# nygenome/Lancet2

Hardware: AMD Instinct MI355X
Metric: microassembly windows/sec (whole node) (higher is better)
Workload: dtype u8/i32 (f64 statistics)

## Files before the change

### lancet2_amd/csrc/build.hip

```cpp
#include "graph_ws.h"

namespace ma {

constexpr int kBT = 256;
__constant__ u64 c_phred_bits[256] = {
#include "../../include/ma_phred_lut.inc"
};

struct SeqInfo {
  u64 off;
  u32 len;
  u32 nk;
};

__device__ __forceinline__ u32 seq_count(const DBatch& b, int w) {
  return 1u + (b.read_win_off[w + 1] - b.read_win_off[w]);
}

__device__ __forceinline__ SeqInfo seq_info(const DBatch& b, int w, u32 s, int k) {
  SeqInfo si;
  if (s == 0) {
    si.off = b.ref_off[w];
    si.len = b.ref_off[w + 1] - b.ref_off[w];
  } else {
// ... 689 lines not shown
      u32 const x = x0 + u * kInsT;
      live[u] = x < nq;
      item[u] = live[u] ? slowq[x] : 0u;
    }
#pragma unroll
    for (int u = 0; u < kIU; ++u) {
      u32 const s_idx = (item[u] >> 12) & kQSeqMask, o = item[u] & 0xFFFu;
      if (staged) {
        off[u] = live[u] ? l_rpos[s_idx] + o : 0u;
        inst[u] = live[u] ? l_ibase[s_idx] + o : 0u;
      } else {
        SeqInfo const si = seq_info(b, w, live[u] ? s_idx : 0u, k);
        off[u] = si.off + o;
        inst[u] = live[u] ? ws.seq_inst_base[base_idx + s_idx] + o : 0u;
      }
    }
#pragma unroll
    for (int u = 0; u < kIU; ++u) {
      id[u] = 1;
      plus[u] = true;
      if (live[u])
        id[u] = staged ? kmer_id_lds(l_seq, static_cast<u32>(off[u]), k, &plus[u]) : kmer_id(b.read_bases + off[u], k, &plus[u]);
    }
#pragma unroll
    for (int u = 0; u < kIU; ++u) {
      if (!live[u]) continue;
      recs[rsi.nk + x0 + u * kInsT] = make_uint4(static_cast<u32>(id[u]), static_cast<u32>(id[u] >> 32),
                                                 inst[u] | (item[u] & (kQErrFree | kQLast)) | (plus[u] ? kQPlus : 0u),
                                                 (item[u] >> 12) & kQSeqMask);
    }
  }
  __threadfence_block();
  __syncthreads();
  IPROF(1);
  auto map_entry = [&](u64 id) -> u32 {
    u32 e = static_cast<u32>(id >> 32) % kInsMap;
    u32 const lim = *reinterpret_cast<volatile u32*>(&l_nmap) + 64u >= kInsMap ? 64u : kInsProbe;
    for (u32 probe = 0; probe < lim; ++probe) {
      u64 cur = l_key[e];
      if (cur == 0) {
        unsigned long long const old = atomicCAS(reinterpret_cast<unsigned long long*>(&l_key[e]), 0ull,
                                                 static_cast<unsigned long long>(id));
        if (old == 0ull) atomicAdd(&l_nmap, 1u);
        cur = old == 0ull ? id : old;
      }
      if (cur == id) return e;
      e = e + 1 == kInsMap ? 0u : e + 1;
    }
    return kNoNode;
  };
  auto map_find = [&](u64 id) -> u32 {
    u32 e = static_cast<u32>(id >> 32) % kInsMap;
    for (u32 probe = 0; probe < kInsProbe; ++probe) {
      u64 const cur = l_key[e];
      if (cur == id) return e;
      if (cur == 0) return kNoNode;
      e = e + 1 == kInsMap ? 0u : e + 1;
    }
    return kNoNode;
  };
  auto const word_flags = [](u32 z) -> u32 {
    return ((z & kQPlus) ? kInstPlus : 0u) | ((z & kQErrFree) ? kInstErrFree : 0u) | ((z & kQLast) ? kInstLast : 0u);
  };
  auto const rec_id = [](uint4 const& r) -> u64 { return static_cast<u64>(r.x) | (static_cast<u64>(r.y) << 32); };
  int const CW = ws.num_samples + 2;
  u32* cnt = ws.tbl_cnt + (static_cast<size_t>(a) << tcl) * CW;
  auto map_pass = [&](u32 ncls, u32 cls) {
    __syncthreads();
    for (u32 i = threadIdx.x; i < kInsMap; i += kInsT) {
      l_key[i] = 0;
      l_min[i] = 0xFFFFFFFFu;
    }
    if (threadIdx.x == 0) l_nmap = 0;
    __syncthreads();
    u32 const sbase = cls * kInsMap;
    for (u32 p = threadIdx.x; p < rsi.nk; p += kInsT) {
      uint4 const rc = recs[p];
      if (ncls > 1 && (rc.x & 0xFFFFu) % ncls != cls) continue;
      u32 const e = map_entry(rec_id(rc));
      if (e != kNoNode) {
        atomicMin(&l_min[e], p);
        inst_slot[p] = (sbase + e) | word_flags(rc.z);
        ref_slot_g[p] = sbase + e;
      } else {
        atomicAdd(&l_ndef, 1u);
      }
    }
    __syncthreads();
    for (u32 x0 = threadIdx.x; x0 < nq; x0 += kInsT * kIU) {
      uint4 rc[kIU];
      bool live[kIU];
#pragma unroll
      for (int u = 0; u < kIU; ++u) {
        u32 const x = x0 + u * kInsT;
        live[u] = x < nq;
        rc[u] = recs[rsi.nk + (live[u] ? x : 0u)];
      }
#pragma unroll
      for (int u = 0; u < kIU; ++u) {
        if (!live[u] || (ncls > 1 && (rc[u].x & 0xFFFFu) % ncls != cls)) continue;
        u32 const e = map_entry(rec_id(rc[u]));
        if (e != kNoNode) {
          u32 const inst = rc[u].z & kInstIdx;
          u32 const before = atomicMin(&l_min[e], inst);
          inst_slot[inst] = (sbase + e) | word_flags(rc[u].z);
          if ((rc[u].z & kQErrFree) && before < rsi.nk) ws.rd_flag[r_first + rc[u].w - 1] = 1;
        } else {
          atomicAdd(&l_ndef, 1u);
        }
      }
    }
    __syncthreads();
  };
  auto copy_out = [&](u32 cls) {
    for (u32 i = threadIdx.x; i < kInsMap; i += kInsT) {
      u64 const id = l_key[i];
      keys[cls * kInsMap + i] = id;
      first[cls * kInsMap + i] = id ? l_min[i] : 0x7F7F7F7Fu;
    }
  };
  map_pass(1, 0);
  IPROF(3);
  if (l_ndef == 0 && (1u << tcl) >= kInsMap) {
    copy_out(0);
    for (u32 i = threadIdx.x; i < kInsMap * CW; i += kInsT) cnt[i] = 0;
    if (threadIdx.x == 0) ws.win_nslots[a] = kInsMap;
    IPROF(4);
    return;
  }
  {
    u32 const ndef0 = l_ndef;
    u32 ncls = 2;
    while (ncls < 16u && (kInsMap + ndef0 / 4u) > ncls * (kInsMap * 6u / 10u)) ncls *= 2u;
    bool tried = false;
    while (ndef0 && ncls <= 16u && (1u << tcl) >= ncls * kInsMap) {
      tried = true;
      __syncthreads();
      if (threadIdx.x == 0) l_ndef = 0;
      for (u32 cls = 0; cls < ncls; ++cls) {
        map_pass(ncls, cls);
        if (l_ndef != 0) break;
        copy_out(cls);
      }
      if (l_ndef == 0) {
        for (u32 i = threadIdx.x; i < ncls * kInsMap * CW; i += kInsT) cnt[i] = 0;
        if (threadIdx.x == 0) ws.win_nslots[a] = ncls * kInsMap;
        return;
      }
      ncls *= 2u;
    }
    if (tried) {
      __syncthreads();
      if (threadIdx.x == 0) l_ndef = 0;
      map_pass(1, 0);
    }
  }
  u32 nslots;
  {
    u32 tcw = 10;
    while (tcw < static_cast<u32>(tcl) && (1u << tcw) < (l_nmap + l_ndef) * 4u / 3u + 16u) ++tcw;
    nslots = 1u << tcw;
  }
  u32 const mask = nslots - 1;
  for (u32 i = threadIdx.x; i < nslots; i += kInsT) {
    keys[i] = 0ull;
    first[i] = 0x7F7F7F7Fu;
  }
  for (u32 i = threadIdx.x; i < nslots * CW; i += kInsT) cnt[i] = 0;
  if (threadIdx.x == 0) ws.win_nslots[a] = nslots;
  __syncthreads();
  for (u32 e = threadIdx.x; e < kInsMap; e += kInsT) {
    u64 const id = l_key[e];
    if (id == 0) continue;
    u32 const slot = table_insert(keys, mask, id, &ws.win_flags[w]);
    u32 const fi = l_min[e];
    if (slot == kNoNode) atomicOr(&ws.win_flags[w], 4u);
    else first[slot] = fi;
    l_min[e] = (slot == kNoNode ? 0x7FFFFFFFu : (slot & kInstSlotMask)) | (fi < rsi.nk ? 0x80000000u : 0u);
  }
  __syncthreads();
  auto direct_insert = [&](u64 id, u32 inst, u32* old_first) -> u32 {
    u32 const slot = table_insert(keys, mask, id, &ws.win_flags[w]);
    *old_first = 0xFFFFFFFFu;
    if (slot == kNoNode) {
      atomicOr(&ws.win_flags[w], 4u);
      return 0u;
    }
    *old_first = atomicMin(&first[slot], inst);
    return slot & kInstSlotMask;
  };
  for (u32 p = threadIdx.x; p < rsi.nk; p += kInsT) {
    uint4 const rc = recs[p];
    u32 const e = map_find(rec_id(rc));
    u32 slot, of;
    if (e != kNoNode) {
      slot = l_min[e] & 0x7FFFFFFFu;
      if (slot == 0x7FFFFFFFu) slot = 0u; else atomicMin(&first[slot], p);
    } else {
      slot = direct_insert(rec_id(rc), p, &of);
    }
    inst_slot[p] = word_flags(rc.z) | slot;
    ref_slot_g[p] = slot;
  }
  __syncthreads();
  for (u32 x = threadIdx.x; x < nq; x += kInsT) {
    uint4 const rc = recs[rsi.nk + x];
    u32 const inst = rc.z & kInstIdx;
    u32 const e = map_find(rec_id(rc));
    u32 slot;
    bool isref;
    if (e != kNoNode) {
      u32 const sv = l_min[e];
      slot = sv & 0x7FFFFFFFu;
      if (slot == 0x7FFFFFFFu) slot = 0u; else atomicMin(&first[slot], inst);
      isref = (sv >> 31) != 0;
    } else {
      u32 of;
      slot = direct_insert(rec_id(rc), inst, &of);
      isref = of < rsi.nk;
    }
    inst_slot[inst] = slot | word_flags(rc.z);
    if ((rc.z & kQErrFree) && isref) ws.rd_flag[r_first + rc.w - 1] = 1;
  }
  IPROF(5);
}
__global__ __launch_bounds__(kInsT) __attribute__((amdgpu_waves_per_eu(8, 8))) void k_insert(DBatch b, GraphWs ws) {
  __shared__ __align__(16) unsigned char l_area[12u * kInsMapA];
  insert_window<kInsMapA, kInsStageA>(b, ws, static_cast<int>(blockIdx.x), l_area);
}
#ifdef MA_PROFILE
extern "C" void ma_debug_iprof(unsigned long long* out) { (void)hipMemcpyFromSymbol(out, HIP_SYMBOL(g_iprof), sizeof(unsigned long long) * 32); }
#endif

constexpr u32 kGrSlots = 6144;
__device__ __forceinline__ u32 edge_word(u32 word) { return ((word & kInstFast) ? (1u << 20) : 0u) | (word & 0xFFFFFu); }
__device__ __forceinline__ uint2 edge_pack(u32 ii, u32 wa, u32 wb) {
  u32 const ca = edge_word(wa), cb = edge_word(wb);
  return make_uint2((ii & 0x3FFFFFu) | (ca << 22), (ca >> 10) | (cb << 11));
}
constexpr u32 kSupCache = 2048;
constexpr int kSupT = 512;
__global__ __launch_bounds__(kSupT) void k_support(DBatch b, GraphWs ws, u32* max_gen, u32 cache_cap, u32 xs_log2) {
  extern __shared__ unsigned char lds_build[];
  __shared__ u32 xs_flag;
  __shared__ u32 any_big;
  __shared__ u32 gen_count;
  __shared__ u32 genq_n;
  __shared__ u32 edgeq_n;
  __shared__ u32 n_leaders;
  int const a = blockIdx.x;
  int const w = static_cast<int>(ws.active[a]);
  int const k = win_kmer(ws, w);
  int const S = ws.num_samples, CW = S + 2;
  u32* gcnt = ws.tbl_cnt + (static_cast<size_t>(a) << tbl_log2(ws)) * CW;
  u32* inst_slot = ws.inst_slot + static_cast<size_t>(a) * ws.inst_stride;
  const u32* ref_slot_g = ws.ref_slot + static_cast<size_t>(a) * ws.ref_stride;
  u32 const ns = seq_count(b, w);
  u32 const base_idx = b.read_win_off[w] + w;
  u32 off = 0;
  u32* l_cnt = reinterpret_cast<u32*>(lds_build + off);
  u32 const cnt_words = (ws.ref_stride * CW + 1u) / 2u;
  off += 4u * cnt_words;
  u32* l_dd = reinterpret_cast<u32*>(lds_build + off);
  off += 4u * (kSupT / 64u) << ws.dd_log2;
  u32* l_mask = reinterpret_cast<u32*>(lds_build + off);
  off += 4u * (ws.max_reads + 2u);
  u32 const xs_cap = 1u << xs_log2, xs_shift = 32u - xs_log2;
  u32* l_xkey = reinterpret_cast<u32*>(lds_build + off);
  off += 4u * xs_cap;
  u32* l_xgrp = reinterpret_cast<u32*>(lds_build + off);
  off += 4u * xs_cap;
  u8* l_xsmp = lds_build + off;
  off = (off + xs_cap + 15u) & ~15u;
  u32* c_meta = reinterpret_cast<u32*>(lds_build + off);
  u32* c_qn = c_meta + cache_cap;
  u32* c_ib = c_qn + cache_cap;
  i32* c_hint = reinterpret_cast<i32*>(c_ib + cache_cap);
  bool const cached = cache_cap != 0 && ns <= cache_cap;
  SeqInfo const rsi = seq_info(b, w, 0, k);
  for (u32 i = threadIdx.x; i < cnt_words; i += kSupT) l_cnt[i] = 0;
  for (u32 i = threadIdx.x; i < (kSupT / 64u) << ws.dd_log2; i += kSupT) l_dd[i] = 0;
  for (u32 i = threadIdx.x; i < xs_cap; i += kSupT) {
    l_xkey[i] = 0;
    l_xgrp[i] = 0;
  }
  if (threadIdx.x == 0) {
    xs_flag = ns > 65535u ? 1u : 0u;
    any_big = 0;
    gen_count = 0;
    genq_n = 0;
    edgeq_n = 0;
  }
  if (cached) {
    for (u32 sx = 1 + threadIdx.x; sx < ns; sx += kSupT) {
      u32 const r = b.read_win_off[w] + sx - 1;
      SeqInfo const si = seq_info(b, w, sx, k);
      c_meta[sx] = (b.read_flags[r] & 7u) | (ws.rd_flag[r] ? 8u : 0u) | (static_cast<u32>(b.read_sample[r]) << 8) | (min(si.nk, 0xFFFFu) << 16);
      c_qn[sx] = b.read_qname_id[r];
      c_ib[sx] = ws.seq_inst_base[base_idx + sx];
      c_hint[sx] = b.read_hint ? b.read_hint[r] : 0;
    }
  }
  __syncthreads();
  bool const hints = b.read_hint != nullptr && rsi.len <= ws.max_ref_len + 8;
  if (hints) {
    for (u32 s_idx = 1 + threadIdx.x; s_idx < ns; s_idx += kSupT) {
      u32 const r = b.read_win_off[w] + s_idx - 1;
      if (!(b.read_flags[r] & MA_RF_PASS)) continue;
      u32 const key = ((b.read_qname_id[r] << 1) | ((b.read_flags[r] & MA_RF_CASE) ? 1u : 0u)) + 1u;
      u32 h = (key * 2654435761u) >> xs_shift;
      bool done = false;
      for (u32 probe = 0; probe < xs_cap && !done; ++probe) {
        u32 cur = l_xkey[h];
        if (cur == 0) {
          u32 const old = atomicCAS(&l_xkey[h], 0u, key);
          if (old == 0) {
            l_xsmp[h] = b.read_sample[r];
            done = true;
            break;
          }
          cur = old;
        }
        if (cur == key) done = true; else h = (h + 1) & (xs_cap - 1);
      }
      if (!done) xs_flag = 1;
    }
  }
  __syncthreads();
  if (hints) {
    for (u32 s_idx = 1 + threadIdx.x; s_idx < ns; s_idx += kSupT) {
      u32 const r = b.read_win_off[w] + s_idx - 1;
      if (!(b.read_flags[r] & MA_RF_PASS)) continue;
      bool const leader = !(s_idx > 1 && same_group(b, r, r - 1));
      u32 const key = ((b.read_qname_id[r] << 1) | ((b.read_flags[r] & MA_RF_CASE) ? 1u : 0u)) + 1u;
      u32 h = (key * 2654435761u) >> xs_shift;
      for (u32 probe = 0; probe < xs_cap; ++probe) {
        u32 const cur = l_xkey[h];
        if (cur == key) {
          if (l_xsmp[h] != b.read_sample[r]) xs_flag = 1;
          if (leader && atomicAdd(&l_xgrp[h], 1u) != 0) xs_flag = 1;
          break;
        }
        if (cur == 0) break;
        h = (h + 1) & (xs_cap - 1);
      }
    }
  }
  if (hints && ns > kSeqCap) {
    for (u32 s_idx = 1 + kMmRunMax + threadIdx.x; s_idx < ns; s_idx += kSupT) {
      u32 const r = b.read_win_off[w] + s_idx - 1;
      u32 j = 0;
      while (j < kMmRunMax && same_group(b, r - j, r - j - 1)) ++j;
      if (j == kMmRunMax) xs_flag = 1;
    }
  }
  __syncthreads();
  bool const all_generic = !hints || xs_flag != 0;
  bool const qmode = !all_generic && !ws.mm_force_hbm && ns <= kSeqCap && tbl_log2(ws) <= 20;
  u32* const genq = ws.slowq + static_cast<size_t>(a) * ws.inst_stride;
  u32 const dd_cap = 1u << ws.dd_log2;
  uint2* const edgeq = reinterpret_cast<uint2*>(ws.slow_rec + static_cast<size_t>(a) * ws.inst_stride);

  u32* const l_leaders = l_mask;
  if (threadIdx.x == 0) n_leaders = 0;
  __syncthreads();
  for (u32 s_idx = 1 + threadIdx.x; s_idx < ns; s_idx += kSupT) {
    u32 const r0 = b.read_win_off[w] + s_idx - 1;
    if (!(b.read_flags[r0] & MA_RF_PASS)) continue;
    if (s_idx > 1 && same_group(b, r0, r0 - 1)) continue;
    l_leaders[atomicAdd(&n_leaders, 1u)] = s_idx;
    if (qmode) {
      u32 tot = 0;
      for (u32 j = 0; s_idx + j < ns && (j == 0 || same_group(b, r0, r0 + j)); ++j) tot += seq_info(b, w, s_idx + j, k).nk;
      if (tot > dd_cap / 4u * 3u) any_big = 1;
    }
  }
  __syncthreads();
  bool const qdedup = qmode && ws.graph_fused && !any_big && ws.win_nslots[a] <= kGrSlots;
  IPROF_T0();
  u32 const wave = threadIdx.x >> 6, lane = threadIdx.x & 63u;
  u32* const dd = l_dd + (wave << ws.dd_log2);
  u32 wave_gen = 0;
  auto same_group_c = [&](u32 sa, u32 sb) {
    u32 const ma_ = c_meta[sa], mb = c_meta[sb];
    return (mb & MA_RF_PASS) && c_qn[sa] == c_qn[sb] && ((ma_ ^ mb) & MA_RF_CASE) == 0 && ((ma_ ^ mb) & 0xFF00u) == 0;
  };
  for (u32 gi = wave; gi < n_leaders; gi += kSupT / 64) {
    u32 const s_idx = l_leaders[gi];
    u32 const r0 = b.read_win_off[w] + s_idx - 1;
    u32 gsize = 1;
    if (cached) {
      while (s_idx + gsize < ns && same_group_c(s_idx, s_idx + gsize)) gsize++;
    } else {
      while (s_idx + gsize < ns && same_group(b, r0, r0 + gsize)) gsize++;
    }
    bool generic = all_generic || gsize > 2;
    for (u32 gm = 0; gm < gsize && !generic; ++gm) {
      if (cached) {
        u32 const mt = c_meta[s_idx + gm];
        if ((mt & 8u) || (mt >> 16) > 32u * kMaskWords) generic = true;
      } else {
        SeqInfo const si = seq_info(b, w, s_idx + gm, k);
        if (ws.rd_flag[r0 + gm] || si.nk > 32u * kMaskWords) generic = true;
      }
    }
    u32 pre00 = 0, pre01 = 0, pre10 = 0, pre11 = 0;
    bool have_pre = cached && gsize <= 2;
    for (u32 gm = 0; gm < gsize && have_pre; ++gm) {
      u32 const nkc = c_meta[s_idx + gm] >> 16;
      if (nkc == 0xFFFFu || nkc > 128u) have_pre = false;
    }
    if (have_pre) {
      u32 const nka = c_meta[s_idx] >> 16, iba = c_ib[s_idx];
      pre00 = lane < nka ? inst_slot[iba + lane] : 0u;
      pre01 = 64u + lane < nka ? inst_slot[iba + 64u + lane] : 0u;
      if (gsize == 2) {
        u32 const nkb = c_meta[s_idx + 1] >> 16, ibb = c_ib[s_idx + 1];
        pre10 = lane < nkb ? inst_slot[ibb + lane] : 0u;
        pre11 = 64u + lane < nkb ? inst_slot[ibb + 64u + lane] : 0u;
      }
    }
    i32 hint0 = 0;
    u32 nk0 = 0;
    unsigned long long m0[kMaskWords / 2];
#pragma unroll
    for (int x = 0; x < kMaskWords / 2; ++x) m0[x] = 0;
    for (u32 gm = 0; gm < gsize; ++gm) {
      u32 const sx = s_idx + gm;
      u32 const r = r0 + gm;
      SeqInfo si;
      u32 ibase, smp, role;
      i32 hint_r;
      if (cached && (c_meta[sx] >> 16) != 0xFFFFu) {
        u32 const mt = c_meta[sx];
        si.nk = mt >> 16;
        ibase = c_ib[sx];
        smp = (mt >> 8) & 0xFFu;
        role = (mt & MA_RF_CASE) ? 1u : 0u;
        hint_r = c_hint[sx];
      } else {
        si = seq_info(b, w, sx, k);
        ibase = ws.seq_inst_base[base_idx + sx];
        smp = b.read_sample[r];
        role = (b.read_flags[r] & MA_RF_CASE) ? 1u : 0u;
        hint_r = hints ? b.read_hint[r] : 0;
      }
      if (si.nk == 0) continue;
      if (smp >= static_cast<u32>(S)) smp = S - 1;
      if (gm == 0) {
        hint0 = hints ? hint_r : 0;
        nk0 = si.nk;
      }
      for (u32 ob = 0; ob < si.nk; ob += 64) {
        u32 const o = ob + lane;
        u32 const word = have_pre ? (gm == 0 ? (ob == 0 ? pre00 : pre01) : (ob == 0 ? pre10 : pre11))
                                  : (o < si.nk ? inst_slot[ibase + o] : 0u);
        {
          u32 const dn = __shfl_down(word, 1, 64);
          u32 first_next;
          if (have_pre) first_next = ob == 0 ? __shfl(gm == 0 ? pre01 : pre11, 0, 64) : 0u;
          else first_next = ob + 64 < si.nk ? inst_slot[ibase + ob + 64] : 0u;
          u32 const nextw = lane == 63 ? first_next : dn;
          bool const pair = o + 1 < si.nk && !((word & kInstFast) && (nextw & kInstFast) &&
                                               (nextw & kInstSlotMask) == (word & kInstSlotMask) + 1u);
          unsigned long long const em = __ballot(pair);
          if (em) {
            u32 eb = 0;
            if (lane == 0) eb = atomicAdd(&edgeq_n, static_cast<u32>(__popcll(em)));
            eb = __shfl(eb, 0, 64);
            if (pair) edgeq[eb + static_cast<u32>(__popcll(em & ((1ull << lane) - 1ull)))] = edge_pack(ibase + o, word, nextw);
          }
        }
        bool const ef = (word & kInstErrFree) != 0;
        bool const to_gen = ef && (generic || !(word & kInstFast));
        u32 const p = word & kInstSlotMask;
        unsigned long long const gmask = __ballot(to_gen);
        if (qdedup) {
          if (gmask) {
            u32 const nslot = to_gen ? ((word & kInstFast) ? ref_slot_g[p] : p) : 0u;
            bool won = false;
            if (to_gen) {
              u32 const tag = gi + 1u, mine = (nslot << 11) | tag;
              u32 h = (nslot * 2654435761u) >> (32u - ws.dd_log2);
              for (;;) {
                u32 cur = dd[h];
                if ((cur & 0x7FFu) != tag) {
                  u32 const old = atomicCAS(&dd[h], cur, mine);
                  if (old == cur) {
                    won = true;
                    break;
                  }
                  cur = old;
                  if ((cur & 0x7FFu) != tag) continue;
                }
                if (cur == mine) break;
                h = (h + 1u) & (dd_cap - 1u);
              }
            }
            unsigned long long const wm = __ballot(won);
            if (wm) {
              u32 qb = 0;
              if (lane == 0) qb = atomicAdd(&genq_n, static_cast<u32>(__popcll(wm)));
              qb = __shfl(qb, 0, 64);
              if (won) genq[qb + static_cast<u32>(__popcll(wm & ((1ull << lane) - 1ull)))] = (nslot << 4) | (smp << 1) | role;
            }
          }
        } else if (qmode) {
          if (gmask) {
            u32 qb = 0;
            if (lane == 0) qb = atomicAdd(&genq_n, static_cast<u32>(__popcll(gmask)));
            qb = __shfl(qb, 0, 64);
            if (to_gen) {
              u32 const nslot = (word & kInstFast) ? ref_slot_g[p] : p;
              genq[qb + static_cast<u32>(__popcll(gmask & ((1ull << lane) - 1ull)))] = ((nslot << 11) | (s_idx - 1u)) + 1u;
            }
          }
        } else if (to_gen) {
          inst_slot[ibase + o] = word | kInstGen;
        }
        wave_gen += static_cast<u32>(__popcll(gmask));
        bool const fast = ef && !to_gen;
        bool dup = false;
        if (gm == 1 && nk0 > 0 && fast) {
          i64 const o0 = static_cast<i64>(p) - hint0;
          if (o0 >= 0 && o0 < static_cast<i64>(nk0)) {
            unsigned long long wd = 0;
#pragma unroll
            for (int x = 0; x < kMaskWords / 2; ++x) wd = (o0 >> 6) == x ? m0[x] : wd;
            dup = (wd >> (o0 & 63)) & 1ull;
          }
        }
        if (gm == 0 && !generic) {
          unsigned long long const cm = __ballot(fast);
#pragma unroll
          for (int x = 0; x < kMaskWords / 2; ++x)
            if (static_cast<int>(ob >> 6) == x) m0[x] = cm;
        }
        if (fast && !dup) {
          u32 const i1 = p * CW + smp, i2 = p * CW + S + role;
          atomicAdd(&l_cnt[i1 >> 1], 1u << ((i1 & 1u) * 16u));
          atomicAdd(&l_cnt[i2 >> 1], 1u << ((i2 & 1u) * 16u));
        }
      }
    }
  }
  if (lane == 0 && wave_gen) atomicAdd(&gen_count, wave_gen);
  IPROF_SYNC(27);
  if (threadIdx.x == 0) {
    bool const lds_ok = !all_generic && !ws.mm_force_hbm && (ns > kSeqCap || gen_count <= 4u * kMmLdsMax) && tbl_log2(ws) <= 20;
    ws.n_edgeq[a] = edgeq_n;
    ws.n_genq[a] = (qmode || qdedup) ? genq_n : 0u;
    ws.mm_mode[a] = qdedup ? (gen_count | 0x20000000u) : qmode ? (gen_count | 0x40000000u) : (gen_count | (lds_ok ? 0u : 0x80000000u));
    atomic_max_lazy(max_gen, gen_count);
    ws.mm_log2[a] = 0;
    if (!qmode && !lds_ok && gen_count) {
      atomic_max_lazy(max_gen + 1, gen_count);
      u32 lg = 10;
      while (lg < 31u && (1ull << lg) < static_cast<u64>(gen_count) * 4u / 3u + 16u) ++lg;
      unsigned long long const bytes = ((12ull << lg) + 255ull) & ~255ull;
      unsigned long long const at = atomicAdd(ws.mm_pool_used, bytes);
      if (at + bytes <= ws.mm_pool_bytes) {
        ws.mm_off[a] = at;
        ws.mm_log2[a] = lg;
      } else {
        atomicOr(&ws.win_flags[w], 4u);
      }
    }
  }
  for (u32 i = threadIdx.x; i < rsi.nk * CW; i += kSupT) {
    u32 const v = (l_cnt[i >> 1] >> ((i & 1u) * 16u)) & 0xFFFFu;
    if (v == 0) continue;
    u32 const p = i / CW, x = i % CW;
    atomicAdd(&gcnt[static_cast<size_t>(ref_slot_g[p]) * CW + x], v);
  }
  IPROF(28);
}

__device__ __forceinline__ u64 mm_key_of(u32 slot, u32 qname, u32 role) {
  return ((static_cast<u64>(slot) << 33) | (static_cast<u64>(qname) << 1) | role) + 1ull;
}
__device__ __forceinline__ u32 inst_table_slot(u32 word, const u32* ref_slot_g) {
  return (word & kInstFast) ? ref_slot_g[word & kInstSlotMask] : (word & kInstSlotMask);
}

__device__ __forceinline__ void mm_hbm_insert(DBatch const& b, GraphWs const& ws, int a, u32* l_base) {
  if (!(ws.mm_mode[a] & 0x80000000u) || ws.mm_log2[a] == 0) return;
  int const w = static_cast<int>(ws.active[a]);
  u32 const mlg = ws.mm_log2[a];
  u32 const mask = (1u << mlg) - 1;
  u64* keys = reinterpret_cast<u64*>(ws.mm_pool + ws.mm_off[a]);
  u32* mins = reinterpret_cast<u32*>(keys + (size_t(1) << mlg));
  const u32* inst_slot = ws.inst_slot + static_cast<size_t>(a) * ws.inst_stride;
  const u32* ref_slot_g = ws.ref_slot + static_cast<size_t>(a) * ws.ref_stride;
  u32 const ns = seq_count(b, w);
  u32 const base_idx = b.read_win_off[w] + w;
  const u32* sbase = stage_seq_bases(ws.seq_inst_base + base_idx, ns, l_base);
  for (u32 i = threadIdx.x; i < (1u << mlg) / 2u; i += kBT) reinterpret_cast<uint4*>(keys)[i] = make_uint4(0, 0, 0, 0);
  for (u32 i = threadIdx.x; i < (1u << mlg) / 4u; i += kBT)
    reinterpret_cast<uint4*>(mins)[i] = make_uint4(0xFFFFFFFFu, 0xFFFFFFFFu, 0xFFFFFFFFu, 0xFFFFFFFFu);
  __threadfence_block();
  __syncthreads();
  u32 const ninst = ws.win_ninst[w], nref = ninst - ws.win_nread_inst[w];
  for (u32 ii = nref + threadIdx.x; ii < ninst; ii += kBT) {
    u32 const v = inst_slot[ii];
    if ((v & (kInstErrFree | kInstGen)) != (kInstErrFree | kInstGen)) continue;
    u32 const s_idx = seq_of(sbase, ns, ii);
    u32 const r = b.read_win_off[w] + s_idx - 1;
    u32 const qn = b.read_qname_id[r];
    u32 const role = (b.read_flags[r] & MA_RF_CASE) ? 1u : 0u;
    u64 const key = mm_key_of(inst_table_slot(v, ref_slot_g), qn, role);
    u32 slot = static_cast<u32>(dev_fmix64(key)) & mask;
    for (u32 probe = 0; probe <= mask; ++probe) {
      u64 cur = keys[slot];
      if (cur != key && cur == 0) {
        unsigned long long old = atomicCAS(reinterpret_cast<unsigned long long*>(&keys[slot]), 0ull,
                                           static_cast<unsigned long long>(key));
        cur = (old == 0ull) ? key : old;
      }
      if (cur == key) {
        atomicMin(&mins[slot], ii);
        break;
      }
      slot = (slot + 1) & mask;
    }
  }
}

__device__ __forceinline__ void mm_hbm_count(DBatch const& b, GraphWs const& ws, int a, u32* l_base) {
  if (!(ws.mm_mode[a] & 0x80000000u) || ws.mm_log2[a] == 0) return;
  int const w = static_cast<int>(ws.active[a]);
  int const S = ws.num_samples, CW = S + 2;
  u32 const mlg = ws.mm_log2[a];
  u32 const mask = (1u << mlg) - 1;
  const u64* keys = reinterpret_cast<const u64*>(ws.mm_pool + ws.mm_off[a]);
  const u32* mins = reinterpret_cast<const u32*>(keys + (size_t(1) << mlg));
  u32* cnt = ws.tbl_cnt + (static_cast<size_t>(a) << tbl_log2(ws)) * CW;
  const u32* inst_slot = ws.inst_slot + static_cast<size_t>(a) * ws.inst_stride;
  const u32* ref_slot_g = ws.ref_slot + static_cast<size_t>(a) * ws.ref_stride;
  u32 const ns = seq_count(b, w);
  u32 const base_idx = b.read_win_off[w] + w;
  const u32* sbase = stage_seq_bases(ws.seq_inst_base + base_idx, ns, l_base);
  __syncthreads();
  u32 const ninst = ws.win_ninst[w], nref = ninst - ws.win_nread_inst[w];
  for (u32 ii = nref + threadIdx.x; ii < ninst; ii += kBT) {
    u32 const v = inst_slot[ii];
    if ((v & (kInstErrFree | kInstGen)) != (kInstErrFree | kInstGen)) continue;
    u32 const s_idx = seq_of(sbase, ns, ii);
    u32 const r = b.read_win_off[w] + s_idx - 1;
    u32 const qn = b.read_qname_id[r];
    u32 const role = (b.read_flags[r] & MA_RF_CASE) ? 1u : 0u;
    u32 sample = b.read_sample[r];
    if (sample >= static_cast<u32>(S)) sample = S - 1;
    u32 const nslot = inst_table_slot(v, ref_slot_g);
    u64 const key = mm_key_of(nslot, qn, role);
    u32 slot = static_cast<u32>(dev_fmix64(key)) & mask;
    for (u32 probe = 0; probe <= mask; ++probe) {
      u64 const cur = keys[slot];
      if (cur == key) break;
      if (cur == 0) {
        slot = kNoNode;
        break;
      }
      slot = (slot + 1) & mask;
    }
    if (slot == kNoNode || mins[slot] != ii) continue;
    atomicAdd(&cnt[static_cast<size_t>(nslot) * CW + sample], 1u);
    atomicAdd(&cnt[static_cast<size_t>(nslot) * CW + S + role], 1u);
  }
}

__global__ __launch_bounds__(kBT) void k_mm_hbm(DBatch b, GraphWs ws) {
  __shared__ u32 l_base[kSeqCap];
  int const a = blockIdx.x;
  if (!(ws.mm_mode[a] & 0x80000000u) || ws.mm_log2[a] == 0) return;
  mm_hbm_insert(b, ws, a, l_base);
  __threadfence_block();
  __syncthreads();
  mm_hbm_count(b, ws, a, l_base);
}

constexpr int kMmT = 1024;
constexpr u32 kMmQueue = 4096;
constexpr u32 kMmAux = kSeqCap + kSeqCap / 2 + kMmQueue;
template <bool kTestProbe>
__global__ __launch_bounds__(kMmT) void k_mm_lds(DBatch b, GraphWs ws) {
  __shared__ u32 l_set[kMmLdsCap];
  __shared__ u32 l_aux[kMmAux];
  __shared__ u32 l_qn;
  constexpr u32 kBlkShift = 7, kBlkCap = 1024;
  __shared__ u16 l_blk[kBlkCap];
  u32* const l_base = l_aux;
// ... 724 lines not shown
  unsigned char* area = lds_build + 2u * kGrSlots + kGrSlots / 8u + ((2u * ws.ref_stride + 15u) & ~15u);
  u32* l_bits = reinterpret_cast<u32*>(area);
  u32* l_base = l_bits + nw;
  u16* l_pref = reinterpret_cast<u16*>(l_base + kSeqCap);
  u32* l_key = reinterpret_cast<u32*>(area);
  u32* l_ok = l_key + kGrSet;
  int const lane = threadIdx.x & 63, wave = threadIdx.x >> 6;
  u32 const ns = seq_count(b, w);
  u32 const base_idx = b.read_win_off[w] + w;

  for (u32 i = threadIdx.x; i < kGrSlots / 2u; i += kGrT) reinterpret_cast<u32*>(l_node)[i] = 0xFFFFFFFFu;
  for (u32 i = threadIdx.x; i < kGrSlots / 32u; i += kGrT) l_sign[i] = 0;
  if (threadIdx.x == 0) l_fail = 0;
  IPROF_T0();
  u32* const l_ctr = reinterpret_cast<u32*>(area);
  u32 const n_cnt = (ws.mm_mode[a] & 0xE0000000u) == 0x20000000u ? ws.n_genq[a] : 0u;
  if (n_cnt) {
    u32 const ctr_words = (tcap * static_cast<u32>(CW) + 1u) / 2u;
    for (u32 i = threadIdx.x; i < ctr_words; i += kGrT) l_ctr[i] = 0;
    __syncthreads();
    const u32* genq = ws.slowq + static_cast<size_t>(a) * ws.inst_stride;
    constexpr int kQU = 4;
    for (u32 q0 = threadIdx.x; q0 < n_cnt; q0 += kGrT * kQU) {
      u32 e[kQU];
#pragma unroll
      for (int u = 0; u < kQU; ++u) e[u] = genq[min(q0 + u * kGrT, n_cnt - 1u)];
#pragma unroll
      for (int u = 0; u < kQU; ++u) {
        if (q0 + u * kGrT >= n_cnt) continue;
        u32 const sl = min(e[u] >> 4, tcap - 1u);
        u32 const i1 = sl * CW + ((e[u] >> 1) & 7u), i2 = sl * CW + S + (e[u] & 1u);
        atomicAdd(&l_ctr[i1 >> 1], 1u << ((i1 & 1u) * 16u));
        atomicAdd(&l_ctr[i2 >> 1], 1u << ((i2 & 1u) * 16u));
      }
    }
    __syncthreads();
  }
  IPROF(22);
  constexpr u32 kPer = kGrSlots / kGrT;
  u32 fi[kPer];
  u32 surv = 0;
#pragma unroll
  for (u32 j = 0; j < kPer; ++j) {
    u32 const s = threadIdx.x + j * kGrT;
    u32 const sc = s < tcap ? s : 0u;
    u64 const ky = keys[sc];
    fi[j] = first[sc];
    u32 total = 0;
    bool any = false, all = true, touched = false;
    for (int i = 0; i < CW; ++i) {
      u32 c = cnt[static_cast<size_t>(sc) * CW + i];
      if (n_cnt) {
        u32 const x = sc * CW + i;
        u32 const add = (l_ctr[x >> 1] >> ((x & 1u) * 16u)) & 0xFFFFu;
        if (add && s < tcap) {
          c += add;
          cnt[static_cast<size_t>(sc) * CW + i] = c;
          touched = true;
        }
      }
      if (i < S) {
        total += c;
        any |= c > 0;
        all &= c <= 1;
      }
    }
    (void)touched;
    bool const remove = (any && all) || total < min_node_cov;
    if (s < tcap && ky != 0 && !remove && fi[j] < ninst) surv |= 1u << j;
  }
  __threadfence_block();
  __syncthreads();
  for (u32 i = threadIdx.x; i < nw; i += kGrT) l_bits[i] = 0;
  const u32* sbase = stage_seq_bases(ws.seq_inst_base + base_idx, ns, l_base);
  __syncthreads();
#pragma unroll
  for (u32 j = 0; j < kPer; ++j)
    if (surv & (1u << j)) atomicOr(&l_bits[fi[j] >> 5], 1u << (fi[j] & 31u));
  IPROF_SYNC(16);
  u32 total_nodes;
  {
    u32 const per = (nw + kGrT - 1u) / kGrT;
    u32 const w0 = threadIdx.x * per;
    u32 mine = 0;
    for (u32 x = 0; x < per; ++x)
      if (w0 + x < nw) mine += __popc(l_bits[w0 + x]);
    u32 inc = mine;
    for (int d = 1; d < 64; d <<= 1) {
      u32 const y = __shfl_up(inc, d);
      if (lane >= d) inc += y;
    }
    if (lane == 63) sh[wave] = inc;
    __syncthreads();
    u32 before = 0, tot = 0;
    for (int x = 0; x < kGrT / 64; ++x) {
      u32 const t = sh[x];
      if (x < wave) before += t;
      tot += t;
    }
    total_nodes = tot;
    u32 run = before + inc - mine;
    if (tot <= kGrSlots)
      for (u32 x = 0; x < per; ++x)
        if (w0 + x < nw) {
          l_pref[w0 + x] = static_cast<u16>(run);
          run += __popc(l_bits[w0 + x]);
        }
  }
  IPROF_SYNC(17);
  if (threadIdx.x == 0) ws.n_nodes[a] = total_nodes;
  if (total_nodes < ws.nc && total_nodes > kGrSlots) return;
  if (total_nodes >= ws.nc) {
    if (threadIdx.x == 0) {
      atomicOr(&ws.win_flags[w], 4u);
      ws.gr_done[a] = 1;
    }
    return;
  }
  u64 const win_read_off0 = b.read_off[b.read_win_off[w]];
#pragma unroll
  for (u32 j = 0; j < kPer; ++j) {
    if (!(surv & (1u << j))) continue;
    u32 const s = threadIdx.x + j * kGrT, ii = fi[j];
    u32 const idx = l_pref[ii >> 5] + __popc(l_bits[ii >> 5] & ((1u << (ii & 31u)) - 1u));
    l_node[s] = static_cast<u16>(idx);
    u32 const v = inst_slot[ii];
    u32 const sq = seq_of(sbase, ns, ii);
    u32 const o = ii - sbase[sq];
    u32 label = 1, srcbit = 0, rel_off = 0;
    if (sq > 0) {
      u32 const r = b.read_win_off[w] + sq - 1;
      label = (b.read_flags[r] & MA_RF_CASE) ? 4u : 2u;
      srcbit = 0x80000000u;
      rel_off = static_cast<u32>(b.read_off[r] - win_read_off0);
    }
    for (int i = 0; i < S; ++i) ws.nd_cnt[(nb + idx) * S + i] = cnt[static_cast<size_t>(s) * CW + i];
    ws.nd_role[(nb + idx) * 2 + 0] = cnt[static_cast<size_t>(s) * CW + S];
    ws.nd_role[(nb + idx) * 2 + 1] = cnt[static_cast<size_t>(s) * CW + S + 1];
    ws.nd_src[nb + idx] = srcbit | (rel_off + o);
    ws.nd_label[nb + idx] = static_cast<u8>(label);
    ws.nd_sign[nb + idx] = (v & kInstPlus) ? 1 : 0;
    ws.nd_nedge[nb + idx] = 0;
    if (v & kInstPlus) atomicOr(&l_sign[idx >> 5], 1u << (idx & 31u));
  }
  IPROF_SYNC(18);
  SeqInfo const rsi = seq_info(b, w, 0, win_kmer(ws, w));
  u32* refn = ws.ref_node + static_cast<size_t>(a) * ws.ref_stride;
  for (u32 p = threadIdx.x; p < ws.ref_stride; p += kGrT) {
    u32 nd = kGrNone;
    if (p < rsi.nk) nd = l_node[min(ref_slot_g[p], kGrSlots - 1u)];
    l_refn[p] = static_cast<u16>(nd);
    refn[p] = nd == kGrNone ? kNoNode : nd;
  }
  for (u32 i = threadIdx.x; i < kGrSet; i += kGrT) {
    l_key[i] = kGrEmpty;
    l_ok[i] = 0xFFFFFFFFu;
  }
  IPROF_SYNC(19);
  auto const h0_of = [&](u32 src) -> u32 { return __umulhi(src * 2654435761u, kGrSet); };
  auto const set_insert = [&](u32 src, u32 val, u32 okey) {
    u32 const key = (src << 15) | val;
    u32 h = h0_of(src);
    for (u32 probe = 0; probe < kGrProbe; ++probe) {
      u32 cur = l_key[h];
      if (cur == kGrEmpty) {
        u32 const old = atomicCAS(&l_key[h], kGrEmpty, key);
        cur = old == kGrEmpty ? key : old;
      }
      if (cur == key) {
        atomicMin(&l_ok[h], okey);
        return;
      }
      h = h + 1u == kGrSet ? 0u : h + 1u;
    }
    l_fail = 1;
  };
  auto const node_of = [&](u32 c) -> u32 {
    return (c >> 20) ? l_refn[min(c & 0xFFFFFu, ws.ref_stride - 1u)] : l_node[min(c & 0xFFFFFu, kGrSlots - 1u)];
  };
  auto const add_edge = [&](u32 ii, u32 ca, u32 cb) {
    u32 const na = node_of(ca), nbn = node_of(cb);
    if (na == kGrNone || nbn == kGrNone) return;
    u32 const sa_minus = ((l_sign[na >> 5] >> (na & 31u)) & 1u) ^ 1u, sb_minus = ((l_sign[nbn >> 5] >> (nbn & 31u)) & 1u) ^ 1u;
    u32 const fwd = (sa_minus << 1) | sb_minus;
    u32 const rev = ((sb_minus ^ 1u) << 1) | (sa_minus ^ 1u);
    set_insert(na, (nbn << 2) | fwd, 2u * ii);
    set_insert(nbn, (na << 2) | rev, 2u * ii + 1u);
  };
  for (u32 p = threadIdx.x; p + 1 < nref; p += kGrT) add_edge(p, edge_word(inst_slot[p]), edge_word(inst_slot[p + 1]));
  {
    const uint2* edgeq = reinterpret_cast<const uint2*>(ws.slow_rec + static_cast<size_t>(a) * ws.inst_stride);
    u32 const neq = ws.n_edgeq[a];
    constexpr int kU = 4;
    for (u32 q0 = threadIdx.x; q0 < neq; q0 += kGrT * kU) {
      uint2 e[kU];
#pragma unroll
      for (int u = 0; u < kU; ++u) e[u] = edgeq[min(q0 + u * kGrT, neq - 1u)];
#pragma unroll
      for (int u = 0; u < kU; ++u)
        if (q0 + u * kGrT < neq) add_edge(e[u].x & 0x3FFFFFu, (e[u].x >> 22) | ((e[u].y & 0x7FFu) << 10), e[u].y >> 11);
    }
  }
  IPROF_SYNC(20);
  if (l_fail) return;
  bool over = false;
  for (u32 i = threadIdx.x; i < kGrSet; i += kGrT) {
    u32 const key = l_key[i];
    if (key == kGrEmpty) continue;
    u32 const src = key >> 15, myok = l_ok[i];
    u32 r = 0, m = 0, h = h0_of(src);
    for (u32 probe = 0; probe < kGrSet; ++probe) {
      u32 const kk = l_key[h];
      if (kk == kGrEmpty) break;
      if ((kk >> 15) == src) {
        ++m;
        r += l_ok[h] < myok;
      }
      h = h + 1u == kGrSet ? 0u : h + 1u;
    }
    if (r < static_cast<u32>(kEdgeCap)) ws.nd_edge[(nb + src) * kEdgeCap + r] = key & 0x7FFFu;
    if (r == 0) ws.nd_nedge[nb + src] = static_cast<u8>(min(m, static_cast<u32>(kEdgeCap)));
    over |= m > static_cast<u32>(kEdgeCap);
  }
  if (over) atomicOr(&ws.win_flags[w], 4u);
  if (threadIdx.x == 0) ws.gr_done[a] = 1;
  IPROF(21);
}

int run_build_pass(ma_ctx* ctx, const DBatch& b, GraphWs& ws, u32* counters_dev, int tc_log2_alloc) {
  if (ws.n_active == 0) return MA_OK;
  int const S = ws.num_samples;
  size_t const A = ws.n_active;
  ws.tc_log2 = tc_log2_alloc;
  ws.max_slow = counters_dev;
  MA_HIP(ctx, hipMemsetAsync(counters_dev, 0, 12, ctx->stream));
  MA_HIP(ctx, hipMemsetAsync(ws.n_slow, 0, 4 * A, ctx->stream));
  MA_HIP(ctx, hipMemsetAsync(ws.mm_pool_used, 0, 8, ctx->stream));
  u32 const tiles_per_win = std::max<u32>(1, (ws.max_reads + 63) / 64);
  u32 const tile_cap = (64 * ws.max_read_len + 32 + 15) & ~15u;
  size_t const lds_c = ((ws.max_ref_len + 8 + 15) & ~15u) + 2048 + 2ull * tile_cap + 2 * 4ull * 64 * classify_mask_words(ws.max_read_len) + 64;
  if (lds_c > 160 * 1024) {
    ma_set_err(ctx, "ma_assemble_batch: reads too long for the LDS-staged classifier");
    return MA_ERR_PARAM;
  }
  if (lds_c > 65536)
    MA_HIP(ctx, hipFuncSetAttribute(reinterpret_cast<const void*>(k_classify), hipFuncAttributeMaxDynamicSharedMemorySize,
                                    static_cast<int>(lds_c)));
  ctx->tic("k_classify");
  hipLaunchKernelGGL(k_classify, dim3(ws.n_active * tiles_per_win), dim3(kClsT), lds_c, ctx->stream, b, ws, counters_dev,
                     tiles_per_win, tile_cap);
  ctx->toc();
  ctx->tic("k_insert");
  hipLaunchKernelGGL(k_insert, dim3(ws.n_active), dim3(kInsT), 0, ctx->stream, b, ws);
  ctx->toc();
  size_t const lds_g = graph_lds_bytes(ws.inst_stride, ws.ref_stride, S);
  ws.graph_fused = (lds_g <= 120u * 1024u && !getenv("MA_NO_GRAPH_FUSE")) ? 1u : 0u;
  ws.dd_log2 = 9;
  while ((1u << ws.dd_log2) / 4u * 3u < 2u * ws.max_read_len && ws.dd_log2 < 12) ++ws.dd_log2;
  u32 const sup_cache = ws.max_reads + 2 <= kSupCache ? ws.max_reads + 2 : 0u;
  u32 xs_log2 = 10;
  while ((1u << xs_log2) < ws.max_reads + 2 && xs_log2 < 14) ++xs_log2;
  auto const sup_lds = [&](u32 lg) {
    return 2ull * ws.ref_stride * (S + 2) + 4 + (size_t(4 * (kSupT / 64)) << ws.dd_log2) + 4ull * (ws.max_reads + 2) + 9ull * (size_t(1) << lg) + 64 +
           16ull * sup_cache + 16;
  };
  while (xs_log2 > 10 && sup_lds(xs_log2) > 159u * 1024u) --xs_log2;
  size_t const lds_s = sup_lds(xs_log2);
  if (lds_s > 65536)
    MA_HIP(ctx, hipFuncSetAttribute(reinterpret_cast<const void*>(k_support), hipFuncAttributeMaxDynamicSharedMemorySize,
                                    static_cast<int>(lds_s)));
  ctx->tic("k_support");
  ws.mm_probe_max = getenv("MA_MM_PROBE_MAX") ? static_cast<u32>(std::max(1, atoi(getenv("MA_MM_PROBE_MAX")))) : kMmLdsCap;
  hipLaunchKernelGGL(k_support, dim3(ws.n_active), dim3(kSupT), lds_s, ctx->stream, b, ws, counters_dev + 1, sup_cache, xs_log2);
  ctx->toc();
  ctx->tic("k_mm_q");
  hipLaunchKernelGGL(k_mm_q<14>, dim3(std::min<u32>(static_cast<u32>(ws.n_active), 512u)), dim3(kMmT), 0, ctx->stream, b, ws);
  ctx->toc();
  if (ws.max_reads + 1u > kSeqCap) {
    ctx->tic("k_mm_lds");
    if (ws.mm_probe_max < kMmLdsCap) hipLaunchKernelGGL(k_mm_lds<true>, dim3(ws.n_active), dim3(kMmT), 0, ctx->stream, b, ws);
    else hipLaunchKernelGGL(k_mm_lds<false>, dim3(ws.n_active), dim3(kMmT), 0, ctx->stream, b, ws);
    ctx->toc();
  }
  ctx->tic("k_mm_hbm");
  hipLaunchKernelGGL(k_mm_hbm, dim3(ws.n_active), dim3(kBT), 0, ctx->stream, b, ws);
  ctx->toc();
  if (getenv("MA_VERBOSE")) {
    std::vector<u32> mm(A);
    u32 max_gen[2] = {0, 0};
    unsigned long long used = 0;
    MA_HIP(ctx, ma_stream_sync(ctx));
    MA_HIP(ctx, hipMemcpy(mm.data(), ws.mm_mode, 4 * A, hipMemcpyDeviceToHost));
    MA_HIP(ctx, hipMemcpy(max_gen, counters_dev + 1, 8, hipMemcpyDeviceToHost));
    MA_HIP(ctx, hipMemcpy(&used, ws.mm_pool_used, 8, hipMemcpyDeviceToHost));
    size_t nfb = 0, big = 0;
    u64 tot = 0;
    for (u32 v : mm) {
      nfb += v >> 31;
      big += (v & 0x1FFFFFFFu) > kMmLdsMax;
      tot += v & 0x1FFFFFFFu;
    }
    fprintf(stderr, "[ma] mate-mer sets: %zu windows, %zu need the HBM set (%zu by size), mean general instances %.0f, max %u / %u; pool %.1f of %.1f MB\n",
            A, nfb, big, static_cast<double>(tot) / static_cast<double>(A), max_gen[0], max_gen[1], used / 1048576.0, ws.mm_pool_bytes / 1048576.0);
  }
  MA_HIP(ctx, hipMemsetAsync(ws.gr_done, 0, 4 * A, ctx->stream));
  if (ws.graph_fused) {
    if (lds_g > 65536)
      MA_HIP(ctx, hipFuncSetAttribute(reinterpret_cast<const void*>(k_graph), hipFuncAttributeMaxDynamicSharedMemorySize,
                                      static_cast<int>(lds_g)));
    ctx->tic("k_graph");
    hipLaunchKernelGGL(k_graph, dim3(ws.n_active), dim3(kGrT), lds_g, ctx->stream, b, ws, static_cast<u32>(ctx->prm.min_node_cov));
    ctx->toc();
  }
  ctx->tic("k_graph_gen");
  hipLaunchKernelGGL(k_graph_gen, dim3(std::min<u32>(static_cast<u32>(ws.n_active), 512u)), dim3(kRankT), 0, ctx->stream, b, ws,
                     static_cast<u32>(ctx->prm.min_node_cov));
  ctx->toc();
  MA_HIP(ctx, hipGetLastError());
  return MA_OK;
}

int run_count_inst(ma_ctx* ctx, const DBatch& b, const GraphWs& ws, int win0, int nwin, u32* maxima_dev) {
  MA_HIP(ctx, hipMemsetAsync(maxima_dev, 0, 32, ctx->stream));
  hipLaunchKernelGGL(k_count_inst, dim3(nwin), dim3(kBT), 0, ctx->stream, b, ws, win0, nwin, maxima_dev);
  MA_HIP(ctx, hipGetLastError());
  return MA_OK;
}

int run_select_active(ma_ctx* ctx, const GraphWs& ws, int win0, int nwin, const u32* gate_approx, u32* win_k,
                      u32* active, u32* n_active_dev) {
  MA_HIP(ctx, hipMemsetAsync(n_active_dev, 0, 8, ctx->stream));
  hipLaunchKernelGGL(k_select_active, dim3((nwin + 255) / 256), dim3(256), 0, ctx->stream, ws, win0, nwin,
                     gate_approx, win_k, active, n_active_dev, ctx->prm.min_k, ctx->prm.max_k, ctx->prm.k_step);
  MA_HIP(ctx, hipGetLastError());
  return MA_OK;
}

}
```

Baseline: 288,200.

## Add wave-level fast path for small read groups in k_support using LDS caches

Adds a specialized per-wave path for read groups of up to two reads with at most 128 k-mers each. It processes instances with ballots, mbcnt prefix offsets and single-lane atomic reservations for edge and generic queues. The reference-slot map is copied into LDS by reusing the hash-key buffer. Read metadata lookups now come from the LDS cache instead of global memory, and readfirstlane marks wave-uniform values. The cost is more code, register pressure and a second pass over leaders for the groups that still need the general path.

```diff
diff --git a/lancet2_amd/csrc/build.hip b/lancet2_amd/csrc/build.hip
--- a/lancet2_amd/csrc/build.hip
+++ b/lancet2_amd/csrc/build.hip
@@ -1015,12 +1015,34 @@
     }
   }
   __syncthreads();
+  auto same_group_c = [&](u32 sa, u32 sb) {
+    u32 const ma_ = c_meta[sa], mb = c_meta[sb];
+    return (mb & MA_RF_PASS) && c_qn[sa] == c_qn[sb] && ((ma_ ^ mb) & MA_RF_CASE) == 0 && ((ma_ ^ mb) & 0xFF00u) == 0;
+  };
+  auto same_group_w = [&](u32 sa, u32 sb) {
+    u32 const r0_ = b.read_win_off[w] - 1;
+    return cached ? same_group_c(sa, sb) : same_group(b, r0_ + sa, r0_ + sb);
+  };
+  auto read_rec = [&](u32 sx, u32& fl, u32& qn, u32& sm) {
+    if (cached) {
+      u32 const mt = c_meta[sx];
+      fl = mt & 7u;
+      qn = c_qn[sx];
+      sm = (mt >> 8) & 0xFFu;
+    } else {
+      u32 const r = b.read_win_off[w] + sx - 1;
+      fl = b.read_flags[r];
+      qn = b.read_qname_id[r];
+      sm = b.read_sample[r];
+    }
+  };
   bool const hints = b.read_hint != nullptr && rsi.len <= ws.max_ref_len + 8;
   if (hints) {
     for (u32 s_idx = 1 + threadIdx.x; s_idx < ns; s_idx += kSupT) {
-      u32 const r = b.read_win_off[w] + s_idx - 1;
-      if (!(b.read_flags[r] & MA_RF_PASS)) continue;
-      u32 const key = ((b.read_qname_id[r] << 1) | ((b.read_flags[r] & MA_RF_CASE) ? 1u : 0u)) + 1u;
+      u32 fl, qn, sm;
+      read_rec(s_idx, fl, qn, sm);
+      if (!(fl & MA_RF_PASS)) continue;
+      u32 const key = ((qn << 1) | ((fl & MA_RF_CASE) ? 1u : 0u)) + 1u;
       u32 h = (key * 2654435761u) >> xs_shift;
       bool done = false;
       for (u32 probe = 0; probe < xs_cap && !done; ++probe) {
@@ -1028,7 +1050,7 @@
         if (cur == 0) {
           u32 const old = atomicCAS(&l_xkey[h], 0u, key);
           if (old == 0) {
-            l_xsmp[h] = b.read_sample[r];
+            l_xsmp[h] = static_cast<u8>(sm);
             done = true;
             break;
           }
@@ -1042,15 +1064,16 @@
   __syncthreads();
   if (hints) {
     for (u32 s_idx = 1 + threadIdx.x; s_idx < ns; s_idx += kSupT) {
-      u32 const r = b.read_win_off[w] + s_idx - 1;
-      if (!(b.read_flags[r] & MA_RF_PASS)) continue;
-      bool const leader = !(s_idx > 1 && same_group(b, r, r - 1));
-      u32 const key = ((b.read_qname_id[r] << 1) | ((b.read_flags[r] & MA_RF_CASE) ? 1u : 0u)) + 1u;
+      u32 fl, qn, sm;
+      read_rec(s_idx, fl, qn, sm);
+      if (!(fl & MA_RF_PASS)) continue;
+      bool const leader = !(s_idx > 1 && same_group_w(s_idx, s_idx - 1));
+      u32 const key = ((qn << 1) | ((fl & MA_RF_CASE) ? 1u : 0u)) + 1u;
       u32 h = (key * 2654435761u) >> xs_shift;
       for (u32 probe = 0; probe < xs_cap; ++probe) {
         u32 const cur = l_xkey[h];
         if (cur == key) {
-          if (l_xsmp[h] != b.read_sample[r]) xs_flag = 1;
+          if (l_xsmp[h] != sm) xs_flag = 1;
           if (leader && atomicAdd(&l_xgrp[h], 1u) != 0) xs_flag = 1;
           break;
         }
@@ -1068,38 +1091,200 @@
     }
   }
   __syncthreads();
-  bool const all_generic = !hints || xs_flag != 0;
-  bool const qmode = !all_generic && !ws.mm_force_hbm && ns <= kSeqCap && tbl_log2(ws) <= 20;
+  auto const uni = [](u32 v) { return static_cast<u32>(__builtin_amdgcn_readfirstlane(static_cast<int>(v))); };
+  bool const all_generic = uni((!hints || xs_flag != 0) ? 1u : 0u) != 0;
+  bool const qmode = uni((!all_generic && !ws.mm_force_hbm && ns <= kSeqCap && tbl_log2(ws) <= 20) ? 1u : 0u) != 0;
   u32* const genq = ws.slowq + static_cast<size_t>(a) * ws.inst_stride;
   u32 const dd_cap = 1u << ws.dd_log2;
   uint2* const edgeq = reinterpret_cast<uint2*>(ws.slow_rec + static_cast<size_t>(a) * ws.inst_stride);
 
   u32* const l_leaders = l_mask;
   if (threadIdx.x == 0) n_leaders = 0;
+  u16* const l_rs = reinterpret_cast<u16*>(l_xkey);
+  bool const rs_lds = uni((cached && tbl_log2(ws) <= 16 && ws.ref_stride <= 4u * xs_cap) ? 1u : 0u) != 0;
+  if (rs_lds)
+    for (u32 i = threadIdx.x; i < ws.ref_stride; i += kSupT) l_rs[i] = i < rsi.nk ? static_cast<u16>(ref_slot_g[i]) : u16(0);
   __syncthreads();
   for (u32 s_idx = 1 + threadIdx.x; s_idx < ns; s_idx += kSupT) {
-    u32 const r0 = b.read_win_off[w] + s_idx - 1;
-    if (!(b.read_flags[r0] & MA_RF_PASS)) continue;
-    if (s_idx > 1 && same_group(b, r0, r0 - 1)) continue;
+    u32 fl, qn, sm;
+    read_rec(s_idx, fl, qn, sm);
+    if (!(fl & MA_RF_PASS)) continue;
+    if (s_idx > 1 && same_group_w(s_idx, s_idx - 1)) continue;
     l_leaders[atomicAdd(&n_leaders, 1u)] = s_idx;
     if (qmode) {
       u32 tot = 0;
-      for (u32 j = 0; s_idx + j < ns && (j == 0 || same_group(b, r0, r0 + j)); ++j) tot += seq_info(b, w, s_idx + j, k).nk;
+      for (u32 j = 0; s_idx + j < ns && (j == 0 || same_group_w(s_idx, s_idx + j)); ++j)
+        tot += cached ? c_meta[s_idx + j] >> 16 : seq_info(b, w, s_idx + j, k).nk;
       if (tot > dd_cap / 4u * 3u) any_big = 1;
     }
   }
   __syncthreads();
-  bool const qdedup = qmode && ws.graph_fused && !any_big && ws.win_nslots[a] <= kGrSlots;
+  bool const qdedup = uni((qmode && ws.graph_fused && !any_big && ws.win_nslots[a] <= kGrSlots) ? 1u : 0u) != 0;
   IPROF_T0();
-  u32 const wave = threadIdx.x >> 6, lane = threadIdx.x & 63u;
+  u32 const wave = uni(threadIdx.x >> 6), lane = threadIdx.x & 63u;
+  u32 const ns_u = uni(ns), n_lead = uni(n_leaders);
+  auto const below = [](unsigned long long m) {
+    return __builtin_amdgcn_mbcnt_hi(static_cast<u32>(m >> 32), __builtin_amdgcn_mbcnt_lo(static_cast<u32>(m), 0u));
+  };
+  auto const same_rec = [](u32 ma_, u32 qa, u32 mb, u32 qb) {
+    return (mb & MA_RF_PASS) && qa == qb && ((ma_ ^ mb) & MA_RF_CASE) == 0 && ((ma_ ^ mb) & 0xFF00u) == 0;
+  };
   u32* const dd = l_dd + (wave << ws.dd_log2);
   u32 wave_gen = 0;
-  auto same_group_c = [&](u32 sa, u32 sb) {
-    u32 const ma_ = c_meta[sa], mb = c_meta[sb];
-    return (mb & MA_RF_PASS) && c_qn[sa] == c_qn[sb] && ((ma_ ^ mb) & MA_RF_CASE) == 0 && ((ma_ ^ mb) & 0xFF00u) == 0;
+  auto const fast_group = [&](u32 s_idx, u32& mta, u32& mtb, u32& fsize) {
+    mta = uni(c_meta[s_idx]);
+    mtb = 0;
+    fsize = 1;
+    if (s_idx + 1 < ns_u) {
+      u32 const qa = uni(c_qn[s_idx]);
+      mtb = uni(c_meta[s_idx + 1]);
+      if (same_rec(mta, qa, mtb, uni(c_qn[s_idx + 1]))) {
+        fsize = 2;
+        if (s_idx + 2 < ns_u && same_rec(mta, qa, uni(c_meta[s_idx + 2]), uni(c_qn[s_idx + 2]))) fsize = 3;
+      }
+    }
+    return fsize <= 2 && (mta >> 16) <= 128u && (fsize < 2 || (mtb >> 16) <= 128u);
   };
-  for (u32 gi = wave; gi < n_leaders; gi += kSupT / 64) {
-    u32 const s_idx = l_leaders[gi];
+  u32 n_general = rs_lds ? 0u : 1u;
+  if (rs_lds) {
+  for (u32 gi = wave; gi < n_lead; gi += kSupT / 64) {
+    u32 const s_idx = uni(l_leaders[gi]);
+    {
+      u32 mta, mtb, fsize;
+      if (!fast_group(s_idx, mta, mtb, fsize)) {
+        ++n_general;
+        continue;
+      }
+      u32 const nka = mta >> 16, nkb = fsize == 2 ? mtb >> 16 : 0u;
+      {
+        bool const generic = all_generic || (((mta | (fsize == 2 ? mtb : 0u)) & 8u) != 0);
+        u32 const iba = uni(c_ib[s_idx]), ibb = fsize == 2 ? uni(c_ib[s_idx + 1]) : 0u;
+        i32 const hint0 = hints ? static_cast<i32>(uni(static_cast<u32>(c_hint[s_idx]))) : 0;
+        u32 const smp = min((mta >> 8) & 0xFFu, static_cast<u32>(S) - 1u), role = (mta & MA_RF_CASE) ? 1u : 0u;
+        u32 wd[4], nx[4];
+        wd[0] = lane < nka ? inst_slot[iba + lane] : 0u;
+        wd[1] = 64u + lane < nka ? inst_slot[iba + 64u + lane] : 0u;
+        wd[2] = lane < nkb ? inst_slot[ibb + lane] : 0u;
+        wd[3] = 64u + lane < nkb ? inst_slot[ibb + 64u + lane] : 0u;
+        asm volatile("" ::"v"(wd[0]), "v"(wd[1]), "v"(wd[2]), "v"(wd[3]));
+        unsigned long long em[4], gk[4], ck[4], m0a = 0, m0b = 0;
+#pragma unroll
+        for (int j = 0; j < 4; ++j) {
+          u32 const nkg = j < 2 ? nka : nkb, ob = (j & 1) * 64u;
+          em[j] = gk[j] = ck[j] = 0;
+          nx[j] = 0;
+          if (ob >= nkg) continue;
+          u32 const o = ob + lane, word = wd[j];
+          u32 const first_next = (j & 1) ? 0u : uni(wd[j | 1]);
+          u32 const dn = __shfl_down(word, 1, 64);
+          u32 const nextw = lane == 63 ? first_next : dn;
+          nx[j] = nextw;
+          bool const pair = o + 1 < nkg && !((word & kInstFast) && (nextw & kInstFast) &&
+                                             (nextw & kInstSlotMask) == (word & kInstSlotMask) + 1u);
+          em[j] = __ballot(pair);
+          bool const ef = (word & kInstErrFree) != 0;
+          bool const to_gen = ef && (generic || !(word & kInstFast));
+          gk[j] = __ballot(to_gen);
+          bool const fast = ef && !to_gen;
+          bool dup = false;
+          if (j < 2) {
+            if (j == 0) m0a = __ballot(fast); else m0b = __ballot(fast);
+          } else if (fast) {
+            i64 const o0 = static_cast<i64>(word & kInstSlotMask) - hint0;
+            if (o0 >= 0 && o0 < static_cast<i64>(nka)) dup = (((o0 >> 6) ? m0b : m0a) >> (o0 & 63)) & 1ull;
+          }
+          ck[j] = __ballot(fast && !dup);
+        }
+        u32 const ne = static_cast<u32>(__popcll(em[0]) + __popcll(em[1]) + __popcll(em[2]) + __popcll(em[3]));
+        if (ne) {
+          u32 eb = 0;
+          if (lane == 0) eb = atomicAdd(&edgeq_n, ne);
+          eb = uni(eb);
+#pragma unroll
+          for (int j = 0; j < 4; ++j) {
+            if ((em[j] >> lane) & 1ull)
+              edgeq[eb + below(em[j])] = edge_pack((j < 2 ? iba : ibb) + (j & 1) * 64u + lane, wd[j], nx[j]);
+            eb += static_cast<u32>(__popcll(em[j]));
+          }
+        }
+        u32 const ng = static_cast<u32>(__popcll(gk[0]) + __popcll(gk[1]) + __popcll(gk[2]) + __popcll(gk[3]));
+        if (ng) {
+          wave_gen += ng;
+          if (qmode) {
+            u32 nsl[4];
+            unsigned long long qk[4];
+#pragma unroll
+            for (int j = 0; j < 4; ++j) {
+              qk[j] = 0;
+              nsl[j] = 0;
+              if (!gk[j]) continue;
+              bool const to_gen = (gk[j] >> lane) & 1ull;
+              u32 const p = wd[j] & kInstSlotMask;
+              u32 const nslot = to_gen ? ((wd[j] & kInstFast) ? static_cast<u32>(l_rs[p]) : p) : 0u;
+              nsl[j] = nslot;
+              if (qdedup) {
+                bool won = false;
+                if (to_gen) {
+                  u32 const tag = gi + 1u, mine = (nslot << 11) | tag;
+                  u32 h = (nslot * 2654435761u) >> (32u - ws.dd_log2);
+                  for (;;) {
+                    u32 cur = dd[h];
+                    if ((cur & 0x7FFu) != tag) {
+                      u32 const old = atomicCAS(&dd[h], cur, mine);
+                      if (old == cur) {
+                        won = true;
+                        break;
+                      }
+                      cur = old;
+                      if ((cur & 0x7FFu) != tag) continue;
+                    }
+                    if (cur == mine) break;
+                    h = (h + 1u) & (dd_cap - 1u);
+                  }
+                }
+                qk[j] = __ballot(won);
+              } else {
+                qk[j] = gk[j];
+              }
+            }
+            u32 const nq = static_cast<u32>(__popcll(qk[0]) + __popcll(qk[1]) + __popcll(qk[2]) + __popcll(qk[3]));
+            if (nq) {
+              u32 qb = 0;
+              if (lane == 0) qb = atomicAdd(&genq_n, nq);
+              qb = uni(qb);
+#pragma unroll
+              for (int j = 0; j < 4; ++j) {
+                if ((qk[j] >> lane) & 1ull)
+                  genq[qb + below(qk[j])] = qdedup ? ((nsl[j] << 4) | (smp << 1) | role) : (((nsl[j] << 11) | (s_idx - 1u)) + 1u);
+                qb += static_cast<u32>(__popcll(qk[j]));
+              }
+            }
+          } else {
+#pragma unroll
+            for (int j = 0; j < 4; ++j)
+              if ((gk[j] >> lane) & 1ull)
+                inst_slot[(j < 2 ? iba : ibb) + (j & 1) * 64u + lane] = wd[j] | kInstGen;
+          }
+        }
+#pragma unroll
+        for (int j = 0; j < 4; ++j) {
+          if ((ck[j] >> lane) & 1ull) {
+            u32 const p = wd[j] & kInstSlotMask;
+            u32 const i1 = p * CW + smp, i2 = p * CW + S + role;
+            atomicAdd(&l_cnt[i1 >> 1], 1u << ((i1 & 1u) * 16u));
+            atomicAdd(&l_cnt[i2 >> 1], 1u << ((i2 & 1u) * 16u));
+          }
+        }
+      }
+    }
+  }
+  }
+  for (u32 gi = wave; n_general != 0 && gi < n_lead; gi += kSupT / 64) {
+    u32 const s_idx = uni(l_leaders[gi]);
+    if (rs_lds) {
+      u32 mta, mtb, fsize;
+      if (fast_group(s_idx, mta, mtb, fsize)) continue;
+    }
     u32 const r0 = b.read_win_off[w] + s_idx - 1;
     u32 gsize = 1;
     if (cached) {
@@ -2430,6 +2615,8 @@
     }
     fprintf(stderr, "[ma] mate-mer sets: %zu windows, %zu need the HBM set (%zu by size), mean general instances %.0f, max %u / %u; pool %.1f of %.1f MB\n",
             A, nfb, big, static_cast<double>(tot) / static_cast<double>(A), max_gen[0], max_gen[1], used / 1048576.0, ws.mm_pool_bytes / 1048576.0);
+    fprintf(stderr, "[ma] k_support: %zu bytes of LDS per workgroup (ref_stride %u, max_reads %u, cache %u, xs_log2 %u)\n", lds_s,
+            ws.ref_stride, ws.max_reads, sup_cache, xs_log2);
   }
   MA_HIP(ctx, hipMemsetAsync(ws.gr_done, 0, 4 * A, ctx->stream));
   if (ws.graph_fused) {
```

Result: faster. 301,600, median of 6 (+4.7%).
